# ictnlp/StreamSpeech

Measured on AMD Instinct MI355X. Metric: real-time factor (RTFx = audio seconds / wall seconds) + utterances/sec, offline S2ST fr-en, higher is better.
Workload: dtype f32

## Files before the change

include/streamspeech_hip.h:

```cpp
#ifndef STREAMSPEECH_HIP_H
#define STREAMSPEECH_HIP_H

#include <stddef.h>
#include <stdint.h>

#ifdef __cplusplus
extern "C" {
#endif

#define SS_ABI_VERSION 2

typedef struct ss_model ss_model;
typedef struct ss_vocoder ss_vocoder;
typedef struct ss_scratch ss_scratch;
typedef struct ss_stream_pool ss_stream_pool;

typedef struct ss_config {
  int32_t input_feat, conv_channels, conv_kernel;
  int32_t enc_dim, enc_ffn, enc_heads, enc_layers, dw_kernel;
  int32_t src_vocab, tgt_vocab;
  int32_t mt_layers, dec_dim, dec_ffn, dec_heads;
  int32_t t2u_layers, unit_layers, unit_vocab, ctc_upsample;
  int32_t pad, eos, unk;
  int32_t max_rel_pos;
// ... 414 lines not shown
int ss_model_set_pack_invariant(ss_model* m, int on);
int ss_model_get_pack_invariant(ss_model* m);
int ss_debug_canon(int mode);

int ss_debug_last_logits(ss_model* m, void* stream, float* d_out, int64_t cap_floats, int* h_rows, int* h_cols);

int ss_op_ffn_fused(void* stream, const float* dX, int ldx, float* dY, int ldy, const float* ln_g, const float* ln_b,
                    const float* dW1, const float* db1, const float* dW2, const float* db2, float alpha,
                    const float* ln2_g, const float* ln2_b, int M, int D, int F);
int ss_debug_ffn(int grid, int row_tiles_per_wave, int enable);
int ss_debug_rtlin(int grid, int enable);
int ss_debug_conv_c64(int enable);
int ss_debug_conv_c256_rows(int rows);
int ss_debug_conv_c32(int enable);
int ss_debug_conv_c16(int enable);
int64_t ss_debug_enc_step_launches(void);
int ss_op_ln_linear(void* stream, const float* dX, int ldx, const float* ln_g, const float* ln_b, const float* dW,
                    const float* dbias, const float* dR, int ldr, float* dC, int ldc, int M, int N, int K, int act, float alpha,
                    int glu);

int ss_debug_force_tile(int bm, int bn, int ks);
int ss_debug_sk_errors(void);
int ss_debug_attention_split(int v);
int ss_debug_attention_q16(int v);
int ss_debug_enc_step_inject_timeout(ss_model* m);
int ss_debug_scratch_audit(ss_scratch* sc, size_t* booked, size_t* held);
int ss_debug_mt_inject_timeout(ss_model* m);

int ss_op_conv_gemm(void* stream, const float* dA, int lda, const float* dW, const float* dbias,
                    const float* dR, int ldr, const float* dR2, int ldr2, float* dC, int ldc,
// ... 2 lines not shown
typedef struct ss_op_conv_args {
  const float* A; const float* W; const float* bias; const float* R; const float* R2; float* C; float* C2;
  int32_t lda, ldc, ldr, ldr2, ldc2;
  int32_t M, N, Cin, taps, dil, stride, pad, in_len, chunk;
  int32_t in_act; float in_slope;
  int32_t act; float act_slope, alpha, div, c2_slope;
  int32_t glu;
  const int32_t* segs; int32_t nseg, max_seg_out;
  int32_t same_rows;
} ss_op_conv_args;
int ss_op_conv_gemm_ex(void* stream, const ss_op_conv_args* a);
int ss_op_conv_gemm_rows(void* stream, const ss_op_conv_args* a, int m_begin, const int32_t* seg_mb, const float* const* seg_A, int canon);
int ss_op_conv_pair(void* stream, const float* dA, int lda, const float* dW1, const float* db1, const float* dW2, const float* db2,
                    float* dC, int ldc, const float* dR2, int ldr2, float div, float* dC2, int ldc2, float c2_slope, int C, int taps,
                    int dil, int M, int in_len, float slope, const int32_t* d_segs, int nseg);
int ss_op_resblock_fused(void* stream, const float* dX, int ldx, const float* const* dW1, const float* const* dB1,
                         const float* const* dW2, const float* const* dB2, const int32_t* dil, float* dY, int ldy, const float* dR2,
                         int ldr2, float div, int C, int taps, int M, float slope, const int32_t* d_segs, int nseg);
int ss_debug_slab(int grid, long long min_rows);
int ss_op_conv_f16(void* stream, const float* dA, const float* dW, const float* dbias, const float* dR, const float* dR2,
                   float* dC, float* dC2, int M, int C, int taps, int dil, int in_act, float in_slope, int act, float div,
                   const int32_t* d_segs, int nseg);
int ss_op_layernorm(void* stream, const float* dx, int ldx, float* dy, int ldy, const float* dg,
                    const float* db, int M, int D, float eps);
int ss_op_attention(void* stream, const float* dQ, int ldq, const float* dK, int ldk, const float* dV,
                    int ldv, float* dO, int ldo, int Tq, int Tk, int H, float scale, int causal,
                    int chunk, const float* dP, int ldp, const float* du, const float* dv);
typedef struct ss_op_attn_args {
  const float* Q; const float* K; const float* V; float* O;
  int32_t ldq, ldk, ldv, ldo;
// ... 108 lines not shown
```

streamspeech_amd/csrc/debug_ops.hip:

```cpp
#include "model_internal.hpp"
#include "ctc_align.hpp"

static int op_bind_wino(GemmArgs& a, void* stream) {
  static thread_local std::map<hipStream_t, DevBuf> wino_tmps;
  DevBuf& wino_tmp = wino_tmps[(hipStream_t)stream];
  const int N = a.N, Cin = a.Cin, taps = a.taps;
  if ((conv_c64w_enabled() && N == 64 && Cin == 64 && taps >= 3 && conv_c64_eligible(a)) ||
      (conv_c128w_enabled() && N == 128 && Cin == 128 && taps >= 3 && a.same_rows && !a.glu) ||
      (conv_c256w_enabled() && N == 256 && Cin == 256 && taps >= 3 && a.same_rows && !a.glu) ||
      (conv_c32w_enabled() && N == 32 && Cin == 32 && taps >= 3 && conv_c32_eligible(a))) {
    RET(wino_tmp.ensure((size_t)N * ((taps + 2) / 3) * 4 * N * sizeof(float)));
    RET(launch_wino_pack(a.W, wino_tmp.f(), N, taps, (hipStream_t)stream));
    a.Wwino = wino_tmp.f();
  }
  return SS_OK;
}

extern "C" int ss_op_conv_gemm(void* stream, const float* dA, int lda, const float* dW, const float* dbias,
                               const float* dR, int ldr, const float* dR2, int ldr2, float* dC, int ldc, int M,
                               int N, int Cin, int taps, int dil, int stride, int pad, int in_len, int chunk,
                               int in_act, float in_slope, int act, float alpha, float div, int glu) {
  GemmArgs a;
  a.A = dA; a.lda = lda; a.W = dW; a.bias = dbias; a.R = dR; a.ldr = ldr; a.R2 = dR2; a.ldr2 = ldr2; a.C = dC; a.ldc = ldc;
  a.M = M; a.N = N; a.Cin = Cin; a.taps = taps; a.dil = dil; a.stride = stride; a.pad = pad; a.in_len = in_len;
// ... 23 lines not shown
                                    const float* const* seg_A, int canon) {
  if (!x || canon < 0 || canon > 2) return SS_ERR_ARG;
  GemmArgs a;
  op_fill_conv(a, x);
  a.m_begin = m_begin; a.seg_mb = seg_mb; a.seg_A = seg_A; a.canon = canon;
  if (a.W && a.N > 0 && a.taps > 0) RET(op_bind_wino(a, stream));
  return launch_conv_gemm(a, (hipStream_t)stream);
}
extern "C" int ss_op_conv_pair(void* stream, const float* dA, int lda, const float* dW1, const float* db1, const float* dW2,
                               const float* db2, float* dC, int ldc, const float* dR2, int ldr2, float div, float* dC2, int ldc2,
                               float c2_slope, int Cch, int taps, int dil, int M, int in_len, float slope, const int32_t* d_segs,
                               int nseg) {
  return launch_conv_pair(dA, lda, dW1, db1, dW2, db2, dC, ldc, dR2, ldr2, div, dC2, ldc2, c2_slope, Cch, taps, dil, M, in_len, slope,
                          d_segs, nseg, (hipStream_t)stream);
}
extern "C" int ss_op_resblock_fused(void* stream, const float* dX, int ldx, const float* const* dW1, const float* const* dB1,
                                    const float* const* dW2, const float* const* dB2, const int32_t* dil, float* dY, int ldy,
                                    const float* dR2, int ldr2, float div, int Cch, int taps, int M, float slope,
                                    const int32_t* d_segs, int nseg) {
  if (!dW1 || !dB1 || !dW2 || !dB2 || !dil) return SS_ERR_ARG;
  return launch_resblock_fused(dX, ldx, dW1, dB1, dW2, dB2, dil, dY, ldy, dR2, ldr2, div, Cch, taps, M, slope, d_segs, nseg,
                               (hipStream_t)stream);
}
extern "C" int ss_debug_slab(int grid, long long min_rows) {
  if (grid < 0) return SS_ERR_ARG;
  slab_debug(grid, min_rows);
  return SS_OK;
}

extern "C" int ss_op_conv_f16(void* stream, const float* dA, const float* dW, const float* dbias, const float* dR, const float* dR2,
// ... 41 lines not shown
  GemmArgs a;
  a.A = dX; a.lda = ldx; a.W = dW; a.bias = dbias; a.R = dR; a.ldr = ldr; a.C = dC; a.ldc = ldc;
  a.M = M; a.N = N; a.Cin = K; a.in_len = M; a.act = act; a.alpha = alpha; a.glu = glu; a.same_rows = 1;
  a.ln_g = ln_g; a.ln_b = ln_b;
  return launch_conv_gemm(a, (hipStream_t)stream);
}
extern "C" int ss_debug_conv_c64(int enable) {
  if (enable == 4 || enable == 5) { conv_c64w_debug(enable == 5); return SS_OK; }
  if (enable == 6 || enable == 7) { conv_c128w_debug(enable == 7); return SS_OK; }
  if (enable == 8 || enable == 9) { conv_c256w_debug(enable == 9); return SS_OK; }
  conv_c64_debug(enable);
  return SS_OK;
}
extern "C" int ss_debug_conv_c256_rows(int rows) { return conv_c256w_rows_debug(rows); }
extern "C" int ss_debug_conv_c32(int enable) {
  if (enable == 4 || enable == 5) { conv_c32w_debug(enable == 5); return SS_OK; }
  conv_c32_debug(enable);
  return SS_OK;
}
extern "C" int ss_debug_conv_c16(int enable) { conv_c16_debug(enable); return SS_OK; }
extern "C" int64_t ss_debug_enc_step_launches(void) { return (int64_t)enc_step_launch_count(); }
extern "C" int ss_debug_scratch_audit(ss_scratch* sc, size_t* booked, size_t* held) {
  if (!sc || !booked || !held) return SS_ERR_ARG;
  size_t sum = 0;
  bool foreign = false;
  for (DevBuf* b : sc->all()) {
    sum += b->bytes;
    if (b->acct != &sc->acct) foreign = true;
  }
  *booked = sc->acct.used;
  *held = sum;
  return foreign ? SS_ERR_ARG : SS_OK;
}
extern "C" int ss_debug_rtlin(int grid, int enable) {
  if (grid < 0) return SS_ERR_ARG;
// ... 195 lines not shown
```

streamspeech_amd/csrc/dispatch.hpp:

```cpp
#pragma once
#include <functional>

namespace ss {

struct Dispatch {
  int attn_no_mfma = 0;
  int attn_q16 = 1;
  int attn_split = 0;
  int c16_off = 0, c32_off = 0, c64_off = 0;
  long long c16_min_rows = 131072, c32_min_rows = 65536, c64_min_rows = 32768;
  int c64w_on = 1, c128w_on = 1, c256w_on = 1, c32w_on = 1;
  int c64w_min_k = 3;
  long long c128w_min_rows = 65536, c256w_min_rows = 32768;
  int c256w_rows = 128;
  int slab_grid_cap = 0;
  int sk_groups = 0;
  int ffn_force_g = 0;
  int ffn_wm = 3, ffn_wm_forced = 0;
  int ffn_fusion = 1;
  int ffn_min_rows = 1000;
  int force_bm = 0, force_bn = 0, force_ks = 0;
  double sk_min_flops = 4e9;
  int no_resblock_fusion = 0, no_pair_fusion = 0;
  int rt_off = 0, rt_min_rows = 193, rt_force_g = 0;
  long long rt_min_units = 4000;
// ... 21 lines not shown
```

streamspeech_amd/csrc/gemm.hip:

```cpp
#include "gemm.hpp"

#include <atomic>
#include <cstdio>
#include <cstdlib>
#include <cstring>
#include <map>
#include <string>
#include <mutex>
#include <tuple>
#include <type_traits>
#include <utility>
#include <vector>

namespace ss {

using f32x4 = __attribute__((ext_vector_type(4))) float;

template <int BM, int BN, int BK, int WM, int WN, int KS, int PD, bool BLK = false>
__global__ __launch_bounds__(256 * KS) void conv_gemm_kernel(const GemmArgs p) {
  static_assert(WM * WN == 4, "4 waves per k-group");
  static_assert(!BLK || KS == 1, "the blocked chain is the KS = 1 form");
  constexpr int LDK = BK + 8;
  constexpr int WTM = BM / WM, WTN = BN / WN;
  constexpr int TM = WTM / 16, TN = WTN / 16;
// ... 569 lines not shown

static int launch_gemv(const GemmArgs& a, hipStream_t stream) {
  const int kq = a.Cin / 256;
  if (a.N * 1 >= 2048 || kq % 2 != 0) return launch_gemv_ks<1>(a, stream);
  if (a.N * 2 >= 2048 || kq % 4 != 0) return launch_gemv_ks<2>(a, stream);
  return launch_gemv_ks<4>(a, stream);
}

static const char* kTileNames[] = {
    "conv_gemm<128,16,16,4,1>", "conv_gemm<128,32,32,4,1>", "conv_gemm<128,32,16,4,1>", "conv_gemm<16,128,32,1,4>",
    "conv_gemm<16,128,16,1,4>", "conv_gemm<128,128,16,2,2>", "conv_gemm<128,64,32,2,2>", "conv_gemm<64,64,32,2,2>",
    "conv_gemm<64,64,16,2,2>", "conv_gemm<32,64,32,2,2>", "conv_gemm<32,64,16,2,2>", "conv_gemm<32,32,32,2,2>",
    "smallm_gemm<4,1>", "smallm_gemm<2,2>", "smallm_gemm<1,4>", "conv_sk<128,BN,32>",
    "conv_slab<32>", "conv_slab<16>", "conv_sk2<256,128,32>", "conv_sk2_bf16x3<256,128,32>",
    "resblock_fused<32>", "resblock_fused<16>", "ffn_fused<256,2048>", "rt_linear<48,256>", "conv_c64<256,64>", "conv_c32<256,32>", "conv_c16<256,16>", "conv_c64w<256,64>", "conv_c128w<256,128>", "conv_c32w<256,32>", "conv_c256w<256,128>", "rt_linear_kb<48,256>",
    "conv_f16<64>", "conv_f16<128>", "conv_f16<256>"};
static_assert(sizeof(kTileNames) / sizeof(kTileNames[0]) == kNumTileCfg, "one name per ProfCls, in enum order");
static std::atomic<int> g_prof_mask{0};
static std::atomic<int> g_prof_mask_hi{0};
static std::vector<ProfRec> g_prof_recs;
static std::vector<std::pair<hipEvent_t, hipEvent_t>> g_prof_pool;
static std::mutex g_prof_mu;

void prof_enable(int cls_mask) { g_prof_mask.store(cls_mask, std::memory_order_relaxed); }
void prof_enable_hi(int cls_mask) { g_prof_mask_hi.store(cls_mask, std::memory_order_relaxed); }
const char* prof_cfg_name(int cls) { return (cls >= 0 && cls < kNumTileCfg) ? kTileNames[cls] : "?"; }
void prof_reset() {
  for (auto& r : g_prof_recs) g_prof_pool.push_back({r.e0, r.e1});
  g_prof_recs.clear();
}
int prof_read_issued(int cls, double* issued) {
// ... 59 lines not shown
int prof_totals(int cls, double* flops, double* bytes, long long* launches) {
  if (cls < 0 || cls >= kNumTileCfg) return SS_ERR_ARG;
  if (flops) *flops = (double)g_prof_totals[cls].flops.load(std::memory_order_relaxed);
  if (bytes) *bytes = (double)g_prof_totals[cls].bytes.load(std::memory_order_relaxed);
  if (launches) *launches = (long long)g_prof_totals[cls].launches.load(std::memory_order_relaxed);
  return SS_OK;
}
static void algo_work(const GemmArgs& a, double& flops, double& bytes) {
  flops = a.algo_flops > 0 ? a.algo_flops : 2.0 * (double)a.M * a.N * a.taps * a.Cin;
  const double ncols = a.glu ? a.N / 2 : a.N;
  bytes = 4.0 * ((double)a.N * a.taps * a.Cin + (a.bias ? a.N : 0) + (double)a.in_len * a.Cin +
                 (double)a.M * ncols * (1 + (a.R ? 1 : 0) + (a.R2 ? 1 : 0)));
  if (a.algo_bytes > 0) bytes = a.algo_bytes;
}

static bool prof_cls_winograd(ProfCls cls) { return cls >= PROF_CONV_C64W && cls <= PROF_CONV_C256W; }

int prof_begin(const GemmArgs& a, hipStream_t stream, ProfCls cls, ProfRec& rec, bool& prof) {
  {
    double fl, by;
    algo_work(a, fl, by);
    g_prof_totals[cls].flops.fetch_add((unsigned long long)(fl + 0.5), std::memory_order_relaxed);
    g_prof_totals[cls].bytes.fetch_add((unsigned long long)(by + 0.5), std::memory_order_relaxed);
    g_prof_totals[cls].launches.fetch_add(1ull, std::memory_order_relaxed);
    if (g_shape_log.load(std::memory_order_relaxed)) {
      std::lock_guard<std::mutex> lk(g_tot_mu);
      if (!g_shapes) { g_shapes = new std::map<ShapeKey, ShapeTot>(); if (getenv("SS_SHAPE_LOG")) atexit(shape_log_dump); }
      const int ops = (a.R ? 1 : 0) | (a.R2 ? 2 : 0) | (a.C2 ? 4 : 0) | (a.in_act != ACT_NONE ? 8 : 0) | (a.act != ACT_NONE ? 16 : 0) | (a.glu ? 32 : 0) | (a.nseg > 0 ? 64 : 0);
      ShapeTot& z = (*g_shapes)[ShapeKey(cls, a.N, a.taps, a.Cin, ops)];
      z.launches += 1; z.rows += a.M; z.flops += fl; z.bytes += by;
    }
// ... 86 lines not shown
  if (w->sync3) (void)hipFree(w->sync3);
  if (w->dbg) (void)hipFree(w->dbg);
  delete w;
}
namespace {
std::mutex g_disp_mu;
std::atomic<unsigned> g_disp_gen{1};
Dispatch env_defaults() {
  Dispatch d;
  auto I = [](const char* k, int dflt) { const char* e = getenv(k); return e ? atoi(e) : dflt; };
  auto L = [](const char* k, long long dflt) { const char* e = getenv(k); return e ? atoll(e) : dflt; };
  d.attn_split = I("SS_ATTN_NO_SPLIT", 0) ? -1 : 0; d.attn_q16 = I("SS_ATTN_Q16", d.attn_q16);
  d.c16_off = I("SS_NO_CONV_C16", 0) ? 1 : 0; d.c32_off = I("SS_NO_CONV_C32", 0) ? 1 : 0; d.c64_off = I("SS_NO_CONV_C64", 0) ? 1 : 0;
  d.c16_min_rows = L("SS_CONV_C16_MIN_ROWS", d.c16_min_rows); d.c32_min_rows = L("SS_CONV_C32_MIN_ROWS", d.c32_min_rows);
  d.c64_min_rows = L("SS_CONV_C64_MIN_ROWS", d.c64_min_rows);
  d.c64w_on = I("SS_CONV_C64_WINOGRAD", 1); d.c128w_on = I("SS_CONV_C128_WINOGRAD", 1); d.c256w_on = I("SS_CONV_C256_WINOGRAD", 1);
  d.c32w_on = I("SS_CONV_C32_WINOGRAD", 1); d.c64w_min_k = I("SS_CONV_C64_WINOGRAD_MIN_K", 3);
  d.c128w_min_rows = L("SS_CONV_C128_MIN_ROWS", d.c128w_min_rows); d.c256w_min_rows = L("SS_CONV_C256_MIN_ROWS", d.c256w_min_rows);
  if (const int r = I("SS_CONV_C256_ROWS", d.c256w_rows); r == 128 || r == 256) d.c256w_rows = r;
  if (getenv("SS_FFN_WM")) { d.ffn_wm = I("SS_FFN_WM", 3); d.ffn_wm_forced = 1; }
  d.ffn_fusion = I("SS_NO_FFN_FUSION", 0) ? 0 : 1; d.ffn_min_rows = I("SS_FFN_MIN_ROWS", d.ffn_min_rows);
  if (getenv("SS_SK_MIN_GFLOP")) d.sk_min_flops = 1e9 * atof(getenv("SS_SK_MIN_GFLOP"));
  d.no_resblock_fusion = I("SS_NO_RESBLOCK_FUSION", 0); d.no_pair_fusion = I("SS_NO_PAIR_FUSION", 0);
  d.rt_off = I("SS_NO_RTLIN", 0) ? 1 : 0; d.rt_min_rows = I("SS_RTLIN_MIN_ROWS", d.rt_min_rows); d.rt_min_units = L("SS_RTLIN_MIN_UNITS", d.rt_min_units);
  d.rt_kb_min_units = L("SS_RTLIN_KB_MIN_UNITS", d.rt_kb_min_units); d.rt_kb_uw = I("SS_RTLIN_KB_UW", d.rt_kb_uw); d.rt_kb_xmap = I("SS_RTLIN_KB_XMAP", d.rt_kb_xmap);
  return d;
}
Dispatch& process_settings() { static Dispatch d = env_defaults(); return d; }
thread_local const Dispatch* t_disp = nullptr;
thread_local CtxDispatch t_disp_own;
// ... 252 lines not shown
```

streamspeech_amd/csrc/gemm.hpp:

```cpp
#pragma once
#include "common.hpp"
#include "dispatch.hpp"

namespace ss {

struct GemmArgs {
  const float* A = nullptr;
  const float* W = nullptr;
  const float* Wwino = nullptr;
  const void* Wf16 = nullptr;
  const float* bias = nullptr;
  const float* R = nullptr;
  const float* R2 = nullptr;
  float* C = nullptr;
  int lda = 0, ldc = 0, ldr = 0, ldr2 = 0;
  int M = 0, N = 0, Cin = 0;
  int taps = 1, dil = 1, stride = 1, pad = 0;
  int in_len = 0;
  int chunk = 0;
  int m_begin = 0;
  int in_act = ACT_NONE;
  float in_slope = 0.1f;
  int act = ACT_NONE;
  float alpha = 1.0f;
// ... 26 lines not shown
};
int canon_mode();
void canon_debug_set(int mode);

enum ProfCls : int {
  PROF_GEMM_128x16x16 = 0, PROF_GEMM_128x32x32 = 1, PROF_GEMM_128x32x16 = 2, PROF_GEMM_16x128x32 = 3, PROF_GEMM_16x128x16 = 4,
  PROF_GEMM_128x128x16 = 5, PROF_GEMM_128x64x32 = 6, PROF_GEMM_64x64x32 = 7, PROF_GEMM_64x64x16 = 8, PROF_GEMM_32x64x32 = 9,
  PROF_GEMM_32x64x16 = 10, PROF_GEMM_32x32x32 = 11,
  PROF_SMALLM_4x1 = 12, PROF_SMALLM_2x2 = 13, PROF_SMALLM_1x4 = 14,
  PROF_CONV_SK = 15, PROF_CONV_SLAB32 = 16, PROF_CONV_SLAB16 = 17, PROF_CONV_SK2 = 18, PROF_CONV_SK2_BF16X3 = 19,
  PROF_RESBLOCK32 = 20, PROF_RESBLOCK16 = 21, PROF_FFN = 22, PROF_RTLIN = 23,
  PROF_CONV_C64 = 24, PROF_CONV_C32 = 25, PROF_CONV_C16 = 26,
  PROF_CONV_C64W = 27, PROF_CONV_C128W = 28, PROF_CONV_C32W = 29, PROF_CONV_C256W = 30,
  PROF_RTLIN_KB = 31,
  PROF_CONV_F16_64 = 32, PROF_CONV_F16_128 = 33, PROF_CONV_F16_256 = 34,
};
constexpr int kNumTileCfg = PROF_CONV_F16_256 + 1;
void prof_enable(int cls_mask);
void prof_enable_hi(int cls_mask);
void prof_reset();
int prof_read(int cls, double* ms_total, double* flops_total, long long* launches, double* bytes_total = nullptr);
const char* prof_cfg_name(int cls);
int prof_totals(int cls, double* flops, double* bytes, long long* launches);
int prof_read_issued(int cls, double* issued_flops_total);
void prof_shape_log(int on);
int prof_shape_dump(char* buf, int cap);

struct ProfRec { hipEvent_t e0, e1; double flops, bytes, issued; int cls; };
int prof_begin(const GemmArgs& a, hipStream_t stream, ProfCls cls, ProfRec& rec, bool& prof);
int prof_end(hipStream_t stream, ProfRec& rec, bool prof);

struct SkWorkspace {
// ... 75 lines not shown
bool conv_c32w_eligible(const GemmArgs& a);
int launch_conv_c32w(const GemmArgs& a, hipStream_t stream);
void conv_c32w_debug(int enable);
bool conv_c32w_enabled();
void conv_c64_debug(int enable);

bool conv_c32_eligible(const GemmArgs& a);
bool conv_c32_enabled();
int launch_conv_c32(const GemmArgs& a, hipStream_t stream);
void conv_c32_debug(int enable);

bool conv_c16_eligible(const GemmArgs& a);
bool conv_c16_enabled();
int launch_conv_c16(const GemmArgs& a, hipStream_t stream);
void conv_c16_debug(int enable);

bool conv_f16_eligible(const GemmArgs& a);
bool conv_f16_geometry_ok(int C, int taps, int dil);
int launch_conv_f16(const GemmArgs& a, hipStream_t stream);
size_t f16_pack_halves(int C, int taps);
int launch_f16_pack(const float* W, void* Wf, int C, int taps, hipStream_t stream);

bool rtlin_eligible(const GemmArgs& a);
bool rtlin_shape_ok(const GemmArgs& a);
int launch_rtlin(const GemmArgs& a, hipStream_t stream);
void rtlin_debug(int grid, int enable);
bool rtlin_kb_shape_ok(const GemmArgs& a);
bool rtlin_kb_eligible(const GemmArgs& a);
int launch_rtlin_kb(const GemmArgs& a, hipStream_t stream);

// ... 17 lines not shown
```

streamspeech_amd/csrc/vocoder.hip:

```cpp
#include "model_internal.hpp"

#include <cstdint>
#include <tuple>


namespace {
struct WinoShared { DevBuf buf; size_t floats = 0; int refs = 0; };
struct WinoKey {
  int dev; const float* blob; uint64_t sig;
  bool operator<(const WinoKey& o) const { return std::tie(dev, blob, sig) < std::tie(o.dev, o.blob, o.sig); }
};
std::mutex g_wino_mu;
std::map<WinoKey, WinoShared> g_wino;
inline uint64_t fnv(uint64_t h, uint64_t v) { for (int i = 0; i < 8; ++i) { h ^= (v >> (8 * i)) & 0xff; h *= 1099511628211ull; } return h; }
uint64_t blob_sig(const ss_vocoder* v, const float* d_blob) {
  const ss_vocoder_config* cfg = &v->cfg;
  uint64_t sig = fnv(fnv(fnv(14695981039346656037ull, (uint64_t)cfg->upsample_initial_channel), (uint64_t)cfg->n_up), (uint64_t)cfg->n_res);
  for (int j = 0; j < cfg->n_res; ++j) sig = fnv(sig, (uint64_t)cfg->resblock_kernel_sizes[j]);
  for (size_t i = 0; i < v->rb_c1.size(); ++i) sig = fnv(fnv(sig, (uint64_t)(v->rb_c1[i].w - d_blob)), (uint64_t)(v->rb_c2[i].w - d_blob));
  return sig;
}
std::mutex g_f16_mu;
std::map<WinoKey, WinoShared> g_f16;
bool f16_stage(int ch) { return ch == 64 || ch == 128 || ch == 256; }
// ... 36 lines not shown
    }
    C = Co;
  }
  v->post = {w.get("voc.post.w", (int64_t)7 * C), w.get("voc.post.b", 1)};
  {
    auto it = w.map.find("voc.spkr.table");
    if (it != w.map.end()) {
      const int64_t per = (int64_t)16 * C0;
      if (it->second.n <= 0 || it->second.n % per || it->second.n / per > INT32_MAX || (C0 & 3)) { scratch_unref(v->sc); delete v; return SS_ERR_ARG; }
      v->spk_table = it->second.p;
      v->n_spk = (int)(it->second.n / per);
    }
  }
  if (!w.missing.empty()) { scratch_unref(v->sc); delete v; return SS_ERR_MISSING_WEIGHT; }
  {
    auto wino_stage = [](int ch) { return ch == 32 || ch == 64 || ch == 128 || ch == 256; };
    size_t need = 0;
    int Cs = C0;
    for (int i = 0; i < cfg->n_up; ++i) {
      Cs /= 2;
      if (wino_stage(Cs)) for (int j = 0; j < cfg->n_res; ++j) need += 6 * (size_t)Cs * ((cfg->resblock_kernel_sizes[j] + 2) / 3) * 4 * Cs;
    }
    if (need) {
      int dev = 0;
      if (hipGetDevice(&dev) != hipSuccess) { scratch_unref(v->sc); delete v; return SS_ERR_HIP; }
      std::lock_guard<std::mutex> lk(g_wino_mu);
      const WinoKey key{dev, d_blob, blob_sig(v, d_blob)};
      WinoShared& sh = g_wino[key];
      const bool fresh = sh.refs == 0;
      if (!fresh && sh.floats != need) { scratch_unref(v->sc); delete v; return SS_ERR_ARG; }
      if (fresh) {
// ... 214 lines not shown
      if (pa) a.C2 = b.bsa;
      a.algo_flops = 2.0 * Ft * scale * C * Co * c.upsample_kernel_sizes[i];
      if (f16 && Co >= 64) a.canon = CANON_SEQ;
      RET(conv(a, scale));
    }
    scale *= st; C = Co;
    RET(on_stage(scale));
    const bool pa_next = (i + 1 < c.n_up) && up_preact(C);
    for (int j = 0; j < c.n_res; ++j) {
      const int kr = c.resblock_kernel_sizes[j];
      int gM = 0, gnseg = 0; const int* gsegs = nullptr;
      geom(scale, gM, gsegs, gnseg);
      static const int c32_min_k = getenv("SS_CONV_C32_MIN_K") ? atoi(getenv("SS_CONV_C32_MIN_K")) : 7;
      static const int c16_min_k = getenv("SS_CONV_C16_MIN_K") ? atoi(getenv("SS_CONV_C16_MIN_K")) : 11;
      const bool per_conv = (c32 && C == 32 && kr >= c32_min_k) || (c16 && C == 16 && kr >= c16_min_k);
      if (!pa && !per_conv && !disp().no_resblock_fusion && resblock_fused_eligible(C, kr, c.resblock_dilations[j], C, C, gnseg, gM)) {
        const float *W1[3], *B1[3], *W2[3], *B2[3];
        for (int dd = 0; dd < 3; ++dd) {
          const int idx = (i * c.n_res + j) * 3 + dd;
          W1[dd] = v->rb_c1[idx].w; B1[dd] = v->rb_c1[idx].b; W2[dd] = v->rb_c2[idx].w; B2[dd] = v->rb_c2[idx].b;
        }
        RET(launch_resblock_fused(b.bs, C, W1, B1, W2, B2, c.resblock_dilations[j], b.bx, C, j > 0 ? b.bx : nullptr, C,
                                  j == c.n_res - 1 ? (float)c.n_res : 0.f, C, kr, gM, 0.1f, gsegs, gnseg, s));
        continue;
      }
      const bool fuse = !pa && !per_conv && !disp().no_pair_fusion && kr == 3 &&
                        conv_pair_eligible(C, kr, c.resblock_dilations[j][2], C, C, gnseg, gM);
      const float* cur = b.bs;
      for (int dd = 0; dd < 3; ++dd) {
        const int idx = (i * c.n_res + j) * 3 + dd;
// ... 459 lines not shown
```

streamspeech_amd/lib.py:

```python
import ctypes as C
import os

_HERE = os.path.dirname(os.path.abspath(__file__))
LIB_PATH = os.environ.get("SS_HIP_LIB") or os.path.join(_HERE, "libstreamspeech_hip.so")


class SSConfig(C.Structure):
    _fields_ = [(n, C.c_int32) for n in (
        "input_feat", "conv_channels", "conv_kernel", "enc_dim", "enc_ffn", "enc_heads", "enc_layers",
        "dw_kernel", "src_vocab", "tgt_vocab", "mt_layers", "dec_dim", "dec_ffn", "dec_heads",
        "t2u_layers", "unit_layers", "unit_vocab", "ctc_upsample", "pad", "eos", "unk",
        "max_rel_pos", "max_tgt_pos")]


class SSVocoderConfig(C.Structure):
    _fields_ = [
        ("num_embeddings", C.c_int32), ("embedding_dim", C.c_int32), ("model_in_dim", C.c_int32),
        ("upsample_initial_channel", C.c_int32),
        ("n_up", C.c_int32), ("upsample_rates", C.c_int32 * 8), ("upsample_kernel_sizes", C.c_int32 * 8),
        ("n_res", C.c_int32), ("resblock_kernel_sizes", C.c_int32 * 4), ("resblock_dilations", (C.c_int32 * 3) * 4),
        ("dur_hidden", C.c_int32), ("dur_kernel", C.c_int32)]


_vp, _i, _f, _i64 = C.c_void_p, C.c_int, C.c_float, C.c_int64
# ... 252 lines not shown
    "ss_prof_read": (_i, [_i, C.POINTER(C.c_double), C.POINTER(C.c_double), C.POINTER(_i64), C.POINTER(C.c_double)]),
    "ss_prof_totals": (_i, [_i, C.POINTER(C.c_double), C.POINTER(C.c_double), C.POINTER(_i64)]),
    "ss_prof_read_issued": (_i, [_i, C.POINTER(C.c_double)]),
    "ss_prof_shape_log": (_i, [_i]),
    "ss_prof_shape_dump": (_i, [C.c_char_p, _i]),
    "ss_prof_num_classes": (_i, []),
    "ss_prof_class_name": (C.c_char_p, [_i]),
    "ss_debug_force_tile": (_i, [_i, _i, _i]),
    "ss_op_ffn_fused": (_i, [_vp, _vp, _i, _vp, _i, _vp, _vp, _vp, _vp, _vp, _vp, _f, _vp, _vp, _i, _i, _i]),
    "ss_debug_ffn": (_i, [_i, _i, _i]),
    "ss_debug_rtlin": (_i, [_i, _i]),
    "ss_debug_conv_c64": (_i, [_i]),
    "ss_debug_conv_c256_rows": (_i, [_i]),
    "ss_debug_conv_c32": (_i, [_i]),
    "ss_debug_conv_c16": (_i, [_i]),
    "ss_debug_enc_step_launches": (_i64, []),
    "ss_debug_scratch_audit": (_i, [_vp, C.POINTER(C.c_size_t), C.POINTER(C.c_size_t)]),
    "ss_op_ln_linear": (_i, [_vp, _vp, _i, _vp, _vp, _vp, _vp, _vp, _i, _vp, _i, _i, _i, _i, _i, _f, _i]),
    "ss_debug_last_logits": (_i, [_vp, _vp, _vp, _i64, C.POINTER(_i), C.POINTER(_i)]),
    "ss_debug_sk_errors": (_i, []),
    "ss_debug_attention_split": (_i, [_i]),
    "ss_debug_attention_q16": (_i, [_i]),
    "ss_op_conv_gemm": (_i, [_vp, _vp, _i, _vp, _vp, _vp, _i, _vp, _i, _vp, _i, _i, _i, _i, _i, _i, _i, _i, _i, _i,
                             _i, _f, _i, _f, _f, _i]),
    "ss_op_conv_gemm_ex": (_i, [_vp, C.POINTER(SSOpConvArgs)]),
    "ss_op_conv_gemm_rows": (_i, [_vp, C.POINTER(SSOpConvArgs), _i, _vp, _vp, _i]),
    "ss_op_conv_pair": (_i, [_vp, _vp, _i, _vp, _vp, _vp, _vp, _vp, _i, _vp, _i, _f, _vp, _i, _f, _i, _i, _i, _i, _i, _f, _vp, _i]),
    "ss_op_resblock_fused": (_i, [_vp, _vp, _i, _vp, _vp, _vp, _vp, _vp, _vp, _i, _vp, _i, _f, _i, _i, _i, _f, _vp, _i]),
    "ss_debug_slab": (_i, [_i, C.c_longlong]),
    "ss_op_conv_f16": (_i, [_vp, _vp, _vp, _vp, _vp, _vp, _vp, _vp, _i, _i, _i, _i, _i, _f, _i, _f, _vp, _i]),
    "ss_op_layernorm": (_i, [_vp, _vp, _i, _vp, _i, _vp, _vp, _i, _i, _f]),
    "ss_op_attention": (_i, [_vp, _vp, _i, _vp, _i, _vp, _i, _vp, _i, _i, _i, _i, _f, _i, _i, _vp, _i, _vp, _vp]),
    "ss_op_attention_ex": (_i, [_vp, C.POINTER(SSOpAttnArgs)]),
    "ss_op_attention_probs": (_i, [_vp, C.POINTER(SSOpAttnProbsArgs)]),
    "ss_op_attention_pool": (_i, [_vp, C.POINTER(SSOpPoolAttnArgs)]),
    "ss_debug_attention_no_mfma": (_i, [_i]),
    "ss_op_dwconv_bn_silu": (_i, [_vp, _vp, _i, _vp, _i, _vp, _i, _vp, _vp, _vp, _vp, _f, _i, _i, _i]),
    "ss_op_dwconv_bn_silu_ex": (_i, [_vp, _vp, _i, _vp, _i, _vp, _i, _vp, _vp, _vp, _vp, _f, _i, _i, _i, _vp, _i, _i]),
    "ss_op_pool_dwconv": (_i, [_vp, _vp, _vp, _i, _vp, _vp, _i, _vp, _vp, _vp, _vp, _f, _i, _vp, _i, _i]),
    "ss_op_pool_gather_rows": (_i, [_vp, _vp, _vp, _vp, _i, _i, _vp, _vp, _i, _i]),
    "ss_op_pool_gather_ids": (_i, [_vp, _vp, _vp, _vp, _i, _vp, _vp, _i, _i]),
    "ss_op_pool_stack_rows": (_i, [_vp, _vp, _vp, _i, _vp, _vp, _i, _i]),
# ... 70 lines not shown
```

Baseline: 6464.

## Add fused Winograd conv-pair kernel for 16-channel vocoder resblocks

Adds a new HIP kernel that runs both convolutions of a HiFi-GAN resblock pair for 16-channel stages in one launch. It uses a Winograd F(2,3)-style transform on MFMA, keeps the intermediate activation in LDS, and keeps pre-packed weights in registers. The vocoder now packs Winograd weights for 16-channel stages and routes eligible resblocks (taps 7 or 11) through this path instead of the existing per-conv or fused resblock kernels. The aim is fewer launches, fewer multiplies and less global traffic for the intermediate tensor. In exchange it adds register and LDS pressure and slightly different rounding from the transform.

After: 6516 (median of 6 runs). No clear change (+0.8%).

```diff
diff --git a/include/streamspeech_hip.h b/include/streamspeech_hip.h
--- a/include/streamspeech_hip.h
+++ b/include/streamspeech_hip.h
@@ -452,6 +452,8 @@
 int ss_debug_conv_c256_rows(int rows);
 int ss_debug_conv_c32(int enable);
 int ss_debug_conv_c16(int enable);
+int ss_debug_conv_c16w(int enable);
+int ss_debug_conv_c16w_block_rows(int taps, int dil);
 int64_t ss_debug_enc_step_launches(void);
 int ss_op_ln_linear(void* stream, const float* dX, int ldx, const float* ln_g, const float* ln_b, const float* dW,
                     const float* dbias, const float* dR, int ldr, float* dC, int ldc, int M, int N, int K, int act, float alpha,
@@ -484,6 +486,9 @@
 int ss_op_conv_pair(void* stream, const float* dA, int lda, const float* dW1, const float* db1, const float* dW2, const float* db2,
                     float* dC, int ldc, const float* dR2, int ldr2, float div, float* dC2, int ldc2, float c2_slope, int C, int taps,
                     int dil, int M, int in_len, float slope, const int32_t* d_segs, int nseg);
+int ss_op_conv_c16w_pair(void* stream, const float* dA, int lda, const float* dW1, const float* db1, const float* dW2, const float* db2,
+                         float* dC, int ldc, const float* dR2, int ldr2, float div, float* dC2, int ldc2, float c2_slope, int C, int taps,
+                         int dil, int M, int in_len, float slope, const int32_t* d_segs, int nseg);
 int ss_op_resblock_fused(void* stream, const float* dX, int ldx, const float* const* dW1, const float* const* dB1,
                          const float* const* dW2, const float* const* dB2, const int32_t* dil, float* dY, int ldy, const float* dR2,
                          int ldr2, float div, int C, int taps, int M, float slope, const int32_t* d_segs, int nseg);
diff --git a/streamspeech_amd/csrc/conv_c16w.hip b/streamspeech_amd/csrc/conv_c16w.hip
--- /dev/null
+++ b/streamspeech_amd/csrc/conv_c16w.hip
@@ -0,0 +1,253 @@
+#include "slab_common.hpp"
+
+namespace ss {
+
+namespace {
+constexpr int CP_C = 16;
+constexpr int CP_LDA = CP_C + 4;
+constexpr int CP_MAXSEG = 256;
+__host__ __device__ constexpr int cp_midr(int dil) { return dil == 1 ? 256 : dil == 3 ? 252 : 250; }
+__host__ __device__ constexpr int cp_bm(int k, int dil) { return cp_midr(dil) - (k - 1); }
+__host__ __device__ constexpr int cp_xr(int k, int dil) { return cp_midr(dil) + dil * (k - 1); }
+__host__ __device__ constexpr int cp_nf(int k) { return 4 * (k / 3) + (k % 3 ? k % 3 + 1 : 0); }
+[[maybe_unused]] __host__ __device__ constexpr int cp_widx(int k, int q) {
+  return q < 4 * (k / 3) ? q : 4 * (k / 3) + (k % 3 == 1 ? 3 * (q - 4 * (k / 3)) : (q - 4 * (k / 3) == 2 ? 3 : q - 4 * (k / 3)));
+}
+}
+
+template <int K>
+__device__ __forceinline__ void cp_load_w(const float* __restrict__ WW, int r, int g, f32x4 (&wf)[cp_nf(K)]) {
+  constexpr int KW = (K + 2) / 3 * 4 * CP_C;
+#pragma unroll
+  for (int q = 0; q < cp_nf(K); ++q) wf[q] = *reinterpret_cast<const f32x4*>(WW + r * KW + cp_widx(K, q) * CP_C + 4 * g);
+}
+
+template <int K, int DIL, bool SWAP>
+__device__ __forceinline__ void cp_contract(const float* pa0, const float* pa1, f32x4 (&wf)[cp_nf(K)], f32x4 (&acc)[4][2],
+                                            const float* __restrict__ WN, int r, int g) {
+  constexpr int GF = K / 3, TAIL = K % 3, KW = (K + 2) / 3 * 4 * CP_C;
+  const float* wn = WN;
+  if constexpr (SWAP) asm volatile("" : "+s"(wn));
+  auto refetch = [&](int q0, int q1) {
+    if constexpr (SWAP) {
+#pragma unroll
+      for (int q = q0; q < q1; ++q) wf[q] = *reinterpret_cast<const f32x4*>(wn + r * KW + cp_widx(K, q) * CP_C + 4 * g);
+      __builtin_amdgcn_sched_barrier(0);
+    }
+  };
+  auto rd = [&](const float* b, int j) -> f32x4 { return *reinterpret_cast<const f32x4*>(b + j * DIL * CP_LDA); };
+  auto mm = [&](int slot, int q, const f32x4 a0, const f32x4 a1) {
+#pragma unroll
+    for (int e = 0; e < 4; ++e) {
+      acc[slot][0] = __builtin_amdgcn_mfma_f32_16x16x4f32(wf[q][e], a0[e], acc[slot][0], 0, 0, 0);
+      acc[slot][1] = __builtin_amdgcn_mfma_f32_16x16x4f32(wf[q][e], a1[e], acc[slot][1], 0, 0, 0);
+    }
+  };
+  f32x4 x0a = rd(pa0, 0), x0b = rd(pa1, 0);
+#pragma unroll
+  for (int grp = 0; grp < GF; ++grp) {
+    const int j = 3 * grp;
+    const f32x4 x1a = rd(pa0, j + 1), x1b = rd(pa1, j + 1), x2a = rd(pa0, j + 2), x2b = rd(pa1, j + 2);
+    const f32x4 x3a = rd(pa0, j + 3), x3b = rd(pa1, j + 3);
+    mm(0, 4 * grp, x0a - x2a, x0b - x2b);
+    mm(1, 4 * grp + 1, x1a + x2a, x1b + x2b);
+    mm(2, 4 * grp + 2, x2a - x1a, x2b - x1b);
+    mm(3, 4 * grp + 3, x1a - x3a, x1b - x3b);
+    x0a = x3a; x0b = x3b;
+    refetch(4 * grp, 4 * grp + 4);
+  }
+  if constexpr (TAIL == 1) {
+    mm(0, 4 * GF, x0a, x0b);
+    mm(3, 4 * GF + 1, rd(pa0, 3 * GF + 1), rd(pa1, 3 * GF + 1));
+    refetch(4 * GF, 4 * GF + 2);
+  }
+  if constexpr (TAIL == 2) {
+    const f32x4 x1a = rd(pa0, 3 * GF + 1), x1b = rd(pa1, 3 * GF + 1), x2a = rd(pa0, 3 * GF + 2), x2b = rd(pa1, 3 * GF + 2);
+    mm(0, 4 * GF, x0a - x1a, x0b - x1b);
+    mm(1, 4 * GF + 1, x1a, x1b);
+    mm(3, 4 * GF + 2, x1a - x2a, x1b - x2b);
+    refetch(4 * GF, 4 * GF + 3);
+  }
+}
+
+template <int K, int DIL>
+__global__ __launch_bounds__(256, 3) void conv_c16w_pair_kernel(const GemmArgs p, const float* __restrict__ WW2, const float* __restrict__ b1) {
+#if __HIP_DEVICE_COMPILE__
+  static_assert(K == 7 || K == 11, "tail groups of one or two taps");
+  constexpr int LDA = CP_LDA, MIDR = cp_midr(DIL), BM = cp_bm(K, DIL), XR = cp_xr(K, DIL), NF = cp_nf(K);
+  constexpr int H2 = (K - 1) / 2, HX = H2 + DIL * (K - 1) / 2;
+  constexpr int NP = (XR * (CP_C / 4) + 255) / 256;
+  constexpr bool HOLD = K == 7;
+  static_assert(MIDR % (2 * DIL) == 0 && MIDR <= 256 && BM % 2 == 0, "whole pairs, two pair tiles per wave");
+  extern __shared__ __attribute__((aligned(16))) float smem[];
+  float* sA = smem;
+  float* sM = sA + XR * LDA;
+  int* s_blk = reinterpret_cast<int*>(sM + MIDR * LDA);
+
+  const int t = threadIdx.x, lane = t & 63;
+  const int wave = __builtin_amdgcn_readfirstlane(t >> 6);
+  const int r = lane & 15, g = lane >> 4;
+
+  SlabWalk<GemmArgs> w(p, s_blk, BM);
+  __syncthreads();
+  const int nblocks = w.nblocks();
+  const float slope = p.in_slope;
+
+  int blk = blockIdx.x;
+  if (blk >= nblocks) return;
+
+  int t1[2], t2[2];
+  bool pv1[2], pv2[2];
+#pragma unroll
+  for (int i = 0; i < 2; ++i) {
+    const int pp = wave * 32 + i * 16 + r;
+    pv1[i] = pp < MIDR / 2;
+    pv2[i] = pp < BM / 2;
+    const int q1 = pv1[i] ? pp : MIDR / 2 - 1, q2 = pv2[i] ? pp : BM / 2 - 1;
+    t1[i] = 2 * DIL * (q1 / DIL) + q1 % DIL;
+    t2[i] = 2 * q2;
+  }
+  const f32x4 bb1 = *reinterpret_cast<const f32x4*>(b1 + 4 * g);
+  f32x4 wf1[NF], wf2[HOLD ? NF : 1];
+  cp_load_w<K>(p.W, r, g, wf1);
+  if constexpr (HOLD) cp_load_w<K>(WW2, r, g, wf2);
+
+  for (; blk < nblocks; blk += gridDim.x) {
+    w.locate(blk, p.in_len);
+    const int m0 = w.m0, seg_lo = w.seg_lo, seg_hi = w.seg_hi;
+    const int m_hi = p.nseg > 0 ? seg_hi : min(seg_hi, p.M);
+    const bool edge = (m0 - HX < seg_lo) || (m0 - HX + XR > seg_hi);
+    {
+      f32x4 pre[NP];
+#pragma unroll
+      for (int u = 0; u < NP; ++u) {
+        const int rho = (t >> 2) + 64 * u;
+        const int gc = min(max(m0 - HX + rho, seg_lo), seg_hi - 1);
+        pre[u] = *reinterpret_cast<const f32x4*>(p.A + (size_t)gc * p.lda + (t & 3) * 4);
+      }
+      float* dst = sA + (t >> 2) * LDA + (t & 3) * 4;
+#pragma unroll
+      for (int u = 0; u < NP; ++u) {
+        const int rho = (t >> 2) + 64 * u;
+        f32x4 v = pre[u];
+        if (edge) {
+          const int gin = m0 - HX + rho;
+          const bool ok = gin >= seg_lo && gin < seg_hi;
+#pragma unroll
+          for (int e = 0; e < 4; ++e) v[e] = ok ? v[e] : 0.f;
+        }
+#pragma unroll
+        for (int e = 0; e < 4; ++e) v[e] = fmaxf(v[e], v[e] * slope);
+        if (rho < XR) *reinterpret_cast<f32x4*>(dst + u * 64 * LDA) = v;
+      }
+    }
+    __syncthreads();
+
+    f32x4 acc[4][2];
+#pragma unroll
+    for (int f = 0; f < 4; ++f) acc[f][0] = acc[f][1] = f32x4{0.f, 0.f, 0.f, 0.f};
+    cp_contract<K, DIL, !HOLD>(sA + t1[0] * LDA + 4 * g, sA + t1[1] * LDA + 4 * g, wf1, acc, WW2, r, g);
+#pragma unroll
+    for (int i = 0; i < 2; ++i) {
+      f32x4 y[2];
+      y[0] = (acc[0][i] + acc[1][i]) + acc[2][i];
+      y[1] = (acc[1][i] - acc[2][i]) - acc[3][i];
+#pragma unroll
+      for (int h = 0; h < 2; ++h) {
+        const int mu = t1[i] + h * DIL;
+        const int gm = m0 - H2 + mu;
+        const bool in_utt = gm >= seg_lo && gm < seg_hi;
+        f32x4 v;
+#pragma unroll
+        for (int e = 0; e < 4; ++e) {
+          const float x = y[h][e] + bb1[e];
+          v[e] = in_utt ? (x > 0.f ? x : x * slope) : 0.f;
+        }
+        if (pv1[i]) *reinterpret_cast<f32x4*>(sM + mu * LDA + 4 * g) = v;
+      }
+    }
+    __syncthreads();
+
+#pragma unroll
+    for (int f = 0; f < 4; ++f) acc[f][0] = acc[f][1] = f32x4{0.f, 0.f, 0.f, 0.f};
+    if constexpr (HOLD) cp_contract<K, 1, false>(sM + t2[0] * LDA + 4 * g, sM + t2[1] * LDA + 4 * g, wf2, acc, nullptr, r, g);
+    else cp_contract<K, 1, true>(sM + t2[0] * LDA + 4 * g, sM + t2[1] * LDA + 4 * g, wf1, acc, p.W, r, g);
+
+    int le = lane;
+    asm volatile("" : "+v"(le));
+    const int cole = (le >> 4) * 4;
+    f32x4 y[4];
+    int mrow[4];
+#pragma unroll
+    for (int i = 0; i < 2; ++i) {
+      y[i * 2] = (acc[0][i] + acc[1][i]) + acc[2][i];
+      y[i * 2 + 1] = (acc[1][i] - acc[2][i]) - acc[3][i];
+      mrow[i * 2] = m0 + t2[i];
+      mrow[i * 2 + 1] = m0 + t2[i] + 1;
+    }
+    f32x4 bb[1] = {f32x4{0.f, 0.f, 0.f, 0.f}};
+    if (p.bias) bb[0] = *reinterpret_cast<const f32x4*>(p.bias + cole);
+    slab_epi_batch(p, y, bb, [&](int q, int n) -> size_t {
+      return (size_t)min(mrow[n], m_hi - 1) * (q == 0 ? p.ldr : p.ldr2) + cole;
+    });
+#pragma unroll
+    for (int q = 0; q < 4; ++q)
+      if (pv2[q / 2] && mrow[q] < m_hi) slab_epi_store(p, mrow[q], cole, y[q]);
+  }
+#endif
+}
+
+void conv_c16w_debug(int enable) { if (enable >= 0) dispatch_edit([enable](Dispatch& d) { d.c16w_off = enable ? 0 : 1; }); }
+bool conv_c16w_enabled() { return !disp().c16w_off; }
+int conv_c16w_block_rows(int taps, int dil) { return cp_bm(taps, dil); }
+
+bool conv_c16w_pair_eligible(int C, int taps, int dil, int lda, int ldc, int nseg, long long M) {
+  return !disp().c16w_off && C == CP_C && (taps == 7 || taps == 11) && (dil == 1 || dil == 3 || dil == 5) && lda == CP_C &&
+         ldc >= CP_C && (ldc & 3) == 0 && nseg >= 0 && nseg <= CP_MAXSEG && M >= disp().c16_min_rows && slab_rows_ok(M);
+}
+
+template <int K, int DIL>
+static int launch_c16w_t(const GemmArgs& a, const float* WW2, const float* b1, hipStream_t stream) {
+  constexpr size_t lds = (size_t)(cp_xr(K, DIL) + cp_midr(DIL)) * CP_LDA * sizeof(float) + (CP_MAXSEG + 2) * sizeof(int);
+  static_assert(3 * lds <= 160 * 1024, "three workgroups per CU");
+  int cus = 0;
+  int rc = device_cus(cus);
+  if (rc != SS_OK) return rc;
+  const int grid = slab_grid(3, cus, a.M, cp_bm(K, DIL), a.nseg);
+  ProfRec rec{}; bool prof = false;
+  rc = prof_begin(a, stream, PROF_CONV_C16W, rec, prof);
+  if (rc != SS_OK) return rc;
+  hipLaunchKernelGGL((conv_c16w_pair_kernel<K, DIL>), dim3(grid), dim3(256), lds, stream, a, WW2, b1);
+  SS_LAUNCH_CHECK();
+  return prof_end(stream, rec, prof);
+}
+
+int launch_conv_c16w_pair(const float* A, int lda, const float* WW1, const float* b1, const float* WW2, const float* b2, float* Cc,
+                          int ldc, const float* R2, int ldr2, float div, float* C2, int ldc2, float c2_slope, int C, int taps,
+                          int dil, int M, int in_len, float slope, const int* segs, int nseg, hipStream_t stream) {
+  if (!conv_c16w_pair_eligible(C, taps, dil, lda, ldc, nseg, M) || !A || !WW1 || !b1 || !WW2 || !b2 || !Cc || A == Cc) return SS_ERR_ARG;
+  if ((R2 && (ldr2 < CP_C || (ldr2 & 3))) || (C2 && (ldc2 < CP_C || (ldc2 & 3))) || (nseg > 0 && !segs) || !(slope > 0.f && slope < 1.f))
+    return SS_ERR_ARG;
+  if (nseg == 0 && in_len < M) return SS_ERR_ARG;
+  auto mis = [](const void* q) { return (reinterpret_cast<uintptr_t>(q) & 15) != 0; };
+  if (mis(A) || mis(Cc) || mis(R2) || mis(C2) || mis(WW1) || mis(WW2) || mis(b1) || mis(b2)) return SS_ERR_ARG;
+  GemmArgs a;
+  a.A = A; a.lda = lda; a.W = WW1; a.bias = b2; a.R = A; a.ldr = lda; a.R2 = R2; a.ldr2 = ldr2; a.div = div;
+  a.C = Cc; a.ldc = ldc; a.C2 = C2; a.ldc2 = ldc2; a.c2_slope = c2_slope;
+  a.M = M; a.N = C; a.Cin = C; a.taps = taps; a.dil = dil; a.stride = 1; a.pad = dil * (taps - 1) / 2; a.in_len = in_len;
+  a.in_act = ACT_LRELU; a.in_slope = slope; a.same_rows = 1; a.segs = segs; a.nseg = nseg;
+  a.algo_flops = 4.0 * (double)M * C * C * taps;
+  a.algo_bytes = 4.0 * (double)M * C * (2 + (R2 ? 1 : 0));
+  const int key = taps * 10 + dil;
+  switch (key) {
+    case 71: return launch_c16w_t<7, 1>(a, WW2, b1, stream);
+    case 73: return launch_c16w_t<7, 3>(a, WW2, b1, stream);
+    case 75: return launch_c16w_t<7, 5>(a, WW2, b1, stream);
+    case 111: return launch_c16w_t<11, 1>(a, WW2, b1, stream);
+    case 113: return launch_c16w_t<11, 3>(a, WW2, b1, stream);
+    case 115: return launch_c16w_t<11, 5>(a, WW2, b1, stream);
+    default: return SS_ERR_ARG;
+  }
+}
+
+}
diff --git a/streamspeech_amd/csrc/debug_ops.hip b/streamspeech_amd/csrc/debug_ops.hip
--- a/streamspeech_amd/csrc/debug_ops.hip
+++ b/streamspeech_amd/csrc/debug_ops.hip
@@ -61,6 +61,20 @@
   return launch_conv_pair(dA, lda, dW1, db1, dW2, db2, dC, ldc, dR2, ldr2, div, dC2, ldc2, c2_slope, Cch, taps, dil, M, in_len, slope,
                           d_segs, nseg, (hipStream_t)stream);
 }
+extern "C" int ss_op_conv_c16w_pair(void* stream, const float* dA, int lda, const float* dW1, const float* db1, const float* dW2,
+                                    const float* db2, float* dC, int ldc, const float* dR2, int ldr2, float div, float* dC2, int ldc2,
+                                    float c2_slope, int Cch, int taps, int dil, int M, int in_len, float slope, const int32_t* d_segs,
+                                    int nseg) {
+  if (!conv_c16w_pair_eligible(Cch, taps, dil, lda, ldc, nseg, M) || !dA || !dW1 || !db1 || !dW2 || !db2 || !dC || dA == dC) return SS_ERR_ARG;
+  static thread_local std::map<hipStream_t, DevBuf> wino_tmps;
+  DevBuf& tmp = wino_tmps[(hipStream_t)stream];
+  const size_t n = (size_t)Cch * ((taps + 2) / 3) * 4 * Cch;
+  RET(tmp.ensure(2 * n * sizeof(float)));
+  RET(launch_wino_pack(dW1, tmp.f(), Cch, taps, (hipStream_t)stream));
+  RET(launch_wino_pack(dW2, tmp.f() + n, Cch, taps, (hipStream_t)stream));
+  return launch_conv_c16w_pair(dA, lda, tmp.f(), db1, tmp.f() + n, db2, dC, ldc, dR2, ldr2, div, dC2, ldc2, c2_slope, Cch, taps, dil, M,
+                               in_len, slope, d_segs, nseg, (hipStream_t)stream);
+}
 extern "C" int ss_op_resblock_fused(void* stream, const float* dX, int ldx, const float* const* dW1, const float* const* dB1,
                                     const float* const* dW2, const float* const* dB2, const int32_t* dil, float* dY, int ldy,
                                     const float* dR2, int ldr2, float div, int Cch, int taps, int M, float slope,
@@ -132,11 +146,15 @@
 }
 extern "C" int ss_debug_conv_c256_rows(int rows) { return conv_c256w_rows_debug(rows); }
 extern "C" int ss_debug_conv_c32(int enable) {
-  if (enable == 4 || enable == 5) { conv_c32w_debug(enable == 5); return SS_OK; }
+  if (enable == 4 || enable == 5) { conv_c32w_debug(enable == 5); conv_c16w_debug(enable == 5); return SS_OK; }
   conv_c32_debug(enable);
   return SS_OK;
 }
 extern "C" int ss_debug_conv_c16(int enable) { conv_c16_debug(enable); return SS_OK; }
+extern "C" int ss_debug_conv_c16w(int enable) { conv_c16w_debug(enable); return SS_OK; }
+extern "C" int ss_debug_conv_c16w_block_rows(int taps, int dil) {
+  return ((taps == 7 || taps == 11) && (dil == 1 || dil == 3 || dil == 5)) ? conv_c16w_block_rows(taps, dil) : 0;
+}
 extern "C" int64_t ss_debug_enc_step_launches(void) { return (int64_t)enc_step_launch_count(); }
 extern "C" int ss_debug_scratch_audit(ss_scratch* sc, size_t* booked, size_t* held) {
   if (!sc || !booked || !held) return SS_ERR_ARG;
diff --git a/streamspeech_amd/csrc/dispatch.hpp b/streamspeech_amd/csrc/dispatch.hpp
--- a/streamspeech_amd/csrc/dispatch.hpp
+++ b/streamspeech_amd/csrc/dispatch.hpp
@@ -9,6 +9,7 @@
   int attn_split = 0;
   int c16_off = 0, c32_off = 0, c64_off = 0;
   long long c16_min_rows = 131072, c32_min_rows = 65536, c64_min_rows = 32768;
+  int c16w_off = 0, c16w_min_k = 7;
   int c64w_on = 1, c128w_on = 1, c256w_on = 1, c32w_on = 1;
   int c64w_min_k = 3;
   long long c128w_min_rows = 65536, c256w_min_rows = 32768;
diff --git a/streamspeech_amd/csrc/gemm.hip b/streamspeech_amd/csrc/gemm.hip
--- a/streamspeech_amd/csrc/gemm.hip
+++ b/streamspeech_amd/csrc/gemm.hip
@@ -607,7 +607,7 @@
     "smallm_gemm<4,1>", "smallm_gemm<2,2>", "smallm_gemm<1,4>", "conv_sk<128,BN,32>",
     "conv_slab<32>", "conv_slab<16>", "conv_sk2<256,128,32>", "conv_sk2_bf16x3<256,128,32>",
     "resblock_fused<32>", "resblock_fused<16>", "ffn_fused<256,2048>", "rt_linear<48,256>", "conv_c64<256,64>", "conv_c32<256,32>", "conv_c16<256,16>", "conv_c64w<256,64>", "conv_c128w<256,128>", "conv_c32w<256,32>", "conv_c256w<256,128>", "rt_linear_kb<48,256>",
-    "conv_f16<64>", "conv_f16<128>", "conv_f16<256>"};
+    "conv_f16<64>", "conv_f16<128>", "conv_f16<256>", "conv_c16w"};
 static_assert(sizeof(kTileNames) / sizeof(kTileNames[0]) == kNumTileCfg, "one name per ProfCls, in enum order");
 static std::atomic<int> g_prof_mask{0};
 static std::atomic<int> g_prof_mask_hi{0};
@@ -697,7 +697,7 @@
   if (a.algo_bytes > 0) bytes = a.algo_bytes;
 }
 
-static bool prof_cls_winograd(ProfCls cls) { return cls >= PROF_CONV_C64W && cls <= PROF_CONV_C256W; }
+static bool prof_cls_winograd(ProfCls cls) { return (cls >= PROF_CONV_C64W && cls <= PROF_CONV_C256W) || cls == PROF_CONV_C16W; }
 
 int prof_begin(const GemmArgs& a, hipStream_t stream, ProfCls cls, ProfRec& rec, bool& prof) {
   {
@@ -814,6 +814,7 @@
   d.c16_off = I("SS_NO_CONV_C16", 0) ? 1 : 0; d.c32_off = I("SS_NO_CONV_C32", 0) ? 1 : 0; d.c64_off = I("SS_NO_CONV_C64", 0) ? 1 : 0;
   d.c16_min_rows = L("SS_CONV_C16_MIN_ROWS", d.c16_min_rows); d.c32_min_rows = L("SS_CONV_C32_MIN_ROWS", d.c32_min_rows);
   d.c64_min_rows = L("SS_CONV_C64_MIN_ROWS", d.c64_min_rows);
+  d.c16w_off = I("SS_NO_CONV_C16W", 0) ? 1 : 0; d.c16w_min_k = I("SS_CONV_C16W_MIN_K", d.c16w_min_k);
   d.c64w_on = I("SS_CONV_C64_WINOGRAD", 1); d.c128w_on = I("SS_CONV_C128_WINOGRAD", 1); d.c256w_on = I("SS_CONV_C256_WINOGRAD", 1);
   d.c32w_on = I("SS_CONV_C32_WINOGRAD", 1); d.c64w_min_k = I("SS_CONV_C64_WINOGRAD_MIN_K", 3);
   d.c128w_min_rows = L("SS_CONV_C128_MIN_ROWS", d.c128w_min_rows); d.c256w_min_rows = L("SS_CONV_C256_MIN_ROWS", d.c256w_min_rows);
diff --git a/streamspeech_amd/csrc/gemm.hpp b/streamspeech_amd/csrc/gemm.hpp
--- a/streamspeech_amd/csrc/gemm.hpp
+++ b/streamspeech_amd/csrc/gemm.hpp
@@ -64,8 +64,9 @@
   PROF_CONV_C64W = 27, PROF_CONV_C128W = 28, PROF_CONV_C32W = 29, PROF_CONV_C256W = 30,
   PROF_RTLIN_KB = 31,
   PROF_CONV_F16_64 = 32, PROF_CONV_F16_128 = 33, PROF_CONV_F16_256 = 34,
-};
-constexpr int kNumTileCfg = PROF_CONV_F16_256 + 1;
+  PROF_CONV_C16W = 35,
+};
+constexpr int kNumTileCfg = PROF_CONV_C16W + 1;
 void prof_enable(int cls_mask);
 void prof_enable_hi(int cls_mask);
 void prof_reset();
@@ -171,6 +172,13 @@
 bool conv_c16_enabled();
 int launch_conv_c16(const GemmArgs& a, hipStream_t stream);
 void conv_c16_debug(int enable);
+bool conv_c16w_pair_eligible(int C, int taps, int dil, int lda, int ldc, int nseg, long long M);
+int launch_conv_c16w_pair(const float* A, int lda, const float* WW1, const float* b1, const float* WW2, const float* b2, float* C,
+                          int ldc, const float* R2, int ldr2, float div, float* C2, int ldc2, float c2_slope, int Cch, int taps,
+                          int dil, int M, int in_len, float slope, const int* segs, int nseg, hipStream_t stream);
+bool conv_c16w_enabled();
+void conv_c16w_debug(int enable);
+int conv_c16w_block_rows(int taps, int dil);
 
 bool conv_f16_eligible(const GemmArgs& a);
 bool conv_f16_geometry_ok(int C, int taps, int dil);
diff --git a/streamspeech_amd/csrc/vocoder.hip b/streamspeech_amd/csrc/vocoder.hip
--- a/streamspeech_amd/csrc/vocoder.hip
+++ b/streamspeech_amd/csrc/vocoder.hip
@@ -74,7 +74,7 @@
   }
   if (!w.missing.empty()) { scratch_unref(v->sc); delete v; return SS_ERR_MISSING_WEIGHT; }
   {
-    auto wino_stage = [](int ch) { return ch == 32 || ch == 64 || ch == 128 || ch == 256; };
+    auto wino_stage = [](int ch) { return ch == 16 || ch == 32 || ch == 64 || ch == 128 || ch == 256; };
     size_t need = 0;
     int Cs = C0;
     for (int i = 0; i < cfg->n_up; ++i) {
@@ -319,6 +319,24 @@
       static const int c32_min_k = getenv("SS_CONV_C32_MIN_K") ? atoi(getenv("SS_CONV_C32_MIN_K")) : 7;
       static const int c16_min_k = getenv("SS_CONV_C16_MIN_K") ? atoi(getenv("SS_CONV_C16_MIN_K")) : 11;
       const bool per_conv = (c32 && C == 32 && kr >= c32_min_k) || (c16 && C == 16 && kr >= c16_min_k);
+      bool c16w = c16 && C == 16 && !pa && conv_c16w_enabled() && kr >= disp().c16w_min_k && !disp().no_resblock_fusion && !disp().no_pair_fusion;
+      for (int dd = 0; dd < 3 && c16w; ++dd) {
+        const int idx = (i * c.n_res + j) * 3 + dd;
+        c16w = v->rb_c1[idx].ww && v->rb_c2[idx].ww && conv_c16w_pair_eligible(C, kr, c.resblock_dilations[j][dd], C, C, gnseg, gM);
+      }
+      if (c16w) {
+        const float* cur = b.bs;
+        for (int dd = 0; dd < 3; ++dd) {
+          const int idx = (i * c.n_res + j) * 3 + dd;
+          float* out = dd == 0 ? b.br : dd == 1 ? b.br2 : b.bx;
+          const float* R2 = (dd == 2 && j > 0) ? b.bx : nullptr;
+          const float div = (dd == 2 && j == c.n_res - 1) ? (float)c.n_res : 0.f;
+          RET(launch_conv_c16w_pair(cur, C, v->rb_c1[idx].ww, v->rb_c1[idx].b, v->rb_c2[idx].ww, v->rb_c2[idx].b, out, C, R2, C, div,
+                                    nullptr, C, 0.1f, C, kr, c.resblock_dilations[j][dd], gM, gM, 0.1f, gsegs, gnseg, s));
+          cur = out;
+        }
+        continue;
+      }
       if (!pa && !per_conv && !disp().no_resblock_fusion && resblock_fused_eligible(C, kr, c.resblock_dilations[j], C, C, gnseg, gM)) {
         const float *W1[3], *B1[3], *W2[3], *B2[3];
         for (int dd = 0; dd < 3; ++dd) {
diff --git a/streamspeech_amd/lib.py b/streamspeech_amd/lib.py
--- a/streamspeech_amd/lib.py
+++ b/streamspeech_amd/lib.py
@@ -290,6 +290,8 @@
     "ss_debug_conv_c256_rows": (_i, [_i]),
     "ss_debug_conv_c32": (_i, [_i]),
     "ss_debug_conv_c16": (_i, [_i]),
+    "ss_debug_conv_c16w": (_i, [_i]),
+    "ss_debug_conv_c16w_block_rows": (_i, [_i, _i]),
     "ss_debug_enc_step_launches": (_i64, []),
     "ss_debug_scratch_audit": (_i, [_vp, C.POINTER(C.c_size_t), C.POINTER(C.c_size_t)]),
     "ss_op_ln_linear": (_i, [_vp, _vp, _i, _vp, _vp, _vp, _vp, _vp, _i, _vp, _i, _i, _i, _i, _i, _f, _i]),
@@ -302,6 +304,7 @@
     "ss_op_conv_gemm_ex": (_i, [_vp, C.POINTER(SSOpConvArgs)]),
     "ss_op_conv_gemm_rows": (_i, [_vp, C.POINTER(SSOpConvArgs), _i, _vp, _vp, _i]),
     "ss_op_conv_pair": (_i, [_vp, _vp, _i, _vp, _vp, _vp, _vp, _vp, _i, _vp, _i, _f, _vp, _i, _f, _i, _i, _i, _i, _i, _f, _vp, _i]),
+    "ss_op_conv_c16w_pair": (_i, [_vp, _vp, _i, _vp, _vp, _vp, _vp, _vp, _i, _vp, _i, _f, _vp, _i, _f, _i, _i, _i, _i, _i, _f, _vp, _i]),
     "ss_op_resblock_fused": (_i, [_vp, _vp, _i, _vp, _vp, _vp, _vp, _vp, _vp, _i, _vp, _i, _f, _i, _i, _i, _f, _vp, _i]),
     "ss_debug_slab": (_i, [_i, C.c_longlong]),
     "ss_op_conv_f16": (_i, [_vp, _vp, _vp, _vp, _vp, _vp, _vp, _vp, _i, _i, _i, _i, _i, _f, _i, _f, _vp, _i]),
```
